# sea-sky-web/Vision-based-Spatio-Temporal-Analysis

Hardware: AMD Instinct MI355X
Metric: multi-cam frames/sec (7-cam→480×1440 BEV) (higher is better)
Workload: dtype f32; 1 GPU; 7-cam 1080x1920 -> resnet50(stride-8 features)+proj C=64 -> IPM warp -> mean -> 480x1440 BEV (BASELINE configs[1]); cameras=7, cameras_per_gpu=7, channels=64, bev_memory_format=NCHW, parallelism=frame-sharded x1 (no collective)

## Files before the change

### include/bev_mi355x.h

```cpp
#ifndef BEV_MI355X_H
#define BEV_MI355X_H

#include <stdint.h>

#ifdef __cplusplus
extern "C" {
#endif

#define BEV_ERR_ARGS (-1)

#define BEV_FUSE_SUM 0
#define BEV_FUSE_MEAN 1
#define BEV_FUSE_MAX 2

int bev_abi_version(void);

const char *bev_build_source_hash(void);

#define BEV_TUNE_CONV_TILE 1
#define BEV_TUNE_WARP_POOL_KB 2
#define BEV_TUNE_WARP_KERNEL 3
#define BEV_TUNE_WARP_BWD_POOL 5
#define BEV_TUNE_CONV_XCD 6
#define BEV_TUNE_CONV_NBUF 7
#define BEV_TUNE_WGRAD_MFMA 8
#define BEV_TUNE_CONV_DMA 9
#define BEV_TUNE_CONV_X6_TILE 10
#define BEV_TUNE_CONV_X6_KERNEL 11
#define BEV_TUNE_CONV_H16_KERNEL 12
#define BEV_TUNE_CONV_PW_SMALL 13
#define BEV_TUNE_DW_RUN 14
#define BEV_TUNE_CONV_X6_NT 16
#define BEV_TUNE_STEM3_STAGE 17
#define BEV_TUNE_WARP_SPAN 19
#define BEV_TUNE_WARP_TILE_BAND 20
#define BEV_TUNE_CONV_H16_BUF 21
#define BEV_TUNE_CONV_X6_STRIP 22
int bev_tune(int knob, int value);


int bev_linspace_f32(double lo, double hi, int n, float *out_host);

int bev_homography_f32(const float *K, const float *G, int n, float *H, void *stream);


int bev_ipm_warp_f32(const float *feats, int64_t sN, int64_t sC, int64_t sH, int64_t sW, const float *Hmat,
                     const float *xs, const float *ys, int N, int C, int Hf, int Wf, float sx, float sy, int Hb,
                     int Wb, float *out, void *stream);

int bev_ipm_warp_fuse_f32(const float *feats, int64_t sN, int64_t sC, int64_t sH, int64_t sW, const float *Hmat,
                          const float *xs, const float *ys, int B, int V, int C, int Hf, int Wf, float sx, float sy,
                          int Hb, int Wb, int mode, float *out, void *stream);
// ... 365 lines not shown
```

### vision-based-spatio-temporal-analysis_amd/bev_native.py

```python
from __future__ import annotations

import collections.abc
import contextlib
import ctypes
import functools
import os
import subprocess
import threading

import torch

HERE = os.path.dirname(os.path.abspath(__file__))
LIB_PATH = os.path.join(HERE, "libbev_mi355x.so")
ABI_VERSION = 18
BEV_ERR_ARGS = -1

FUSE_MODES = {"sum": 0, "mean": 1, "max": 2}

_lib = None

_vp = ctypes.c_void_p
_i = ctypes.c_int
_i64 = ctypes.c_int64
_f = ctypes.c_float
# ... 233 lines not shown
TUNE_CONV_XCD = 6
TUNE_CONV_NBUF = 7
TUNE_WGRAD_MFMA = 8
TUNE_CONV_DMA = 9
TUNE_CONV_X6_TILE = 10
TUNE_CONV_X6_KERNEL = 11
TUNE_CONV_H16_KERNEL = 12
TUNE_CONV_PW_SMALL = 13
TUNE_DW_RUN = 14
TUNE_CONV_X6_NT = 16
TUNE_STEM3_STAGE = 17
TUNE_WARP_SPAN = 19
TUNE_WARP_TILE_BAND = 20
TUNE_CONV_H16_BUF = 21
TUNE_CONV_X6_STRIP = 22
WARP_KERNEL_DMA, WARP_KERNEL_REGISTER = 0, 1


def tune(knob: int, value: int) -> int:
    rc = lib().bev_tune(knob, value)
    if rc < 0:
        raise ValueError(f"bad tuning knob/value {knob}/{value}")
    return rc


@contextlib.contextmanager
def tuned(**knobs):
    old = []
    try:
        for name, value in knobs.items():
# ... 1910 lines not shown
```

### vision-based-spatio-temporal-analysis_amd/csrc/bev_conv.hip

```cpp
#include <hip/hip_runtime.h>
#include <stdint.h>
#include <stdlib.h>

#include <type_traits>

#include "../../include/bev_mi355x.h"
#include "bev_act.h"
#include "bev_mfma.h"
#include "bev_tune.h"

namespace {

constexpr int BK = 32;
constexpr int LROW = BK + 4;

typedef float f32x16 __attribute__((ext_vector_type(16)));
typedef float f32x2 __attribute__((ext_vector_type(2)));
typedef float f32x4 __attribute__((ext_vector_type(4)));

__device__ __attribute__((aligned(16))) float g_zero4[4] = {0.f, 0.f, 0.f, 0.f};

__host__ __device__ inline int64_t kpad(int K) { return (K + BK - 1) / BK * BK; }
__host__ __device__ inline int64_t copad(int Co) { return (Co + 127) / 128 * 128; }

// ... 1258 lines not shown
    a.xcd = conv_xcd();
    return a;
}

}

extern "C" {

int bev_tune(int knob, int value) {
    if (knob == BEV_TUNE_CONV_TILE) return bev::swap_knob(g_conv_tile, value, 4);
    if (knob == BEV_TUNE_CONV_DMA) return bev::swap_knob(g_conv_dma, value, 2);
    if (knob == BEV_TUNE_CONV_XCD) return bev::swap_knob(g_conv_xcd, value, 1);
    if (knob == BEV_TUNE_CONV_NBUF) return bev::swap_knob(g_conv_nbuf, value, 2);
    if (knob == BEV_TUNE_WGRAD_MFMA) return bev::train_tune(knob, value);
    if (knob == BEV_TUNE_CONV_X6_TILE || knob == BEV_TUNE_CONV_X6_KERNEL || knob == BEV_TUNE_CONV_X6_NT ||
        knob == BEV_TUNE_CONV_X6_STRIP)
        return bev::conv_x6_tune(knob, value);
    if (knob == BEV_TUNE_CONV_H16_KERNEL) return bev::conv_h16_tune(value);
    if (knob == BEV_TUNE_CONV_H16_BUF) return bev::conv_h16_buf_tune(value);
    if (knob == BEV_TUNE_DW_RUN) return bev::dw_tune(value);
    if (knob == BEV_TUNE_STEM3_STAGE) return bev::stem3_tune(value);
    if (knob == BEV_TUNE_CONV_PW_SMALL) return bev::swap_knob(g_conv_pw_small, value, 4);
    return bev::warp_tune(knob, value);
}

int64_t bev_conv_packed_size(int Co, int Ci, int KH, int KW) {
    if (Co <= 0 || Ci <= 0 || KH <= 0 || KW <= 0) return 0;
    return copad(Co) * kpad(Ci * KH * KW);
}

int bev_conv_pack_weights_f32(const float *w, int Co, int Ci, int KH, int KW, float *packed, void *stream) {
// ... 237 lines not shown
```

### vision-based-spatio-temporal-analysis_amd/csrc/bev_conv_x6.hip

```cpp
#include <hip/hip_runtime.h>
#include <stdint.h>

#include <type_traits>

#include "../../include/bev_mi355x.h"
#include "bev_act.h"
#include "bev_mfma.h"
#include "bev_tune.h"

namespace {

typedef __bf16 bf16x8 __attribute__((ext_vector_type(8)));
typedef __bf16 bf16x4 __attribute__((ext_vector_type(4)));
typedef float f32x16 __attribute__((ext_vector_type(16)));
typedef float f32x4 __attribute__((ext_vector_type(4)));
typedef unsigned u32x4 __attribute__((ext_vector_type(4)));
typedef unsigned u32x2 __attribute__((ext_vector_type(2)));

constexpr int XBK = 16;
constexpr int XROW = 24;

__device__ __attribute__((aligned(16))) float g_xzero4[4] = {0.f, 0.f, 0.f, 0.f};

__host__ __device__ inline int64_t kpad_x(int K) { return (K + XBK - 1) / XBK * XBK; }
__host__ __device__ inline int64_t copad_x(int Co) { return (Co + 127) / 128 * 128; }

__device__ __forceinline__ void split3(float v, __bf16 &h, __bf16 &m, __bf16 &l) {
    h = (__bf16)v;
    const float r = v - (float)h;
    m = (__bf16)r;
    l = (__bf16)(r - (float)m);
}

__device__ __forceinline__ void x6_dot(f32x16 &c, const bf16x8 (&a)[3], const bf16x8 (&b)[3]) {
    c = __builtin_amdgcn_mfma_f32_32x32x16_bf16(a[0], b[0], c, 0, 0, 0);
    c = __builtin_amdgcn_mfma_f32_32x32x16_bf16(a[0], b[1], c, 0, 0, 0);
    c = __builtin_amdgcn_mfma_f32_32x32x16_bf16(a[1], b[0], c, 0, 0, 0);
    c = __builtin_amdgcn_mfma_f32_32x32x16_bf16(a[0], b[2], c, 0, 0, 0);
    c = __builtin_amdgcn_mfma_f32_32x32x16_bf16(a[2], b[0], c, 0, 0, 0);
    c = __builtin_amdgcn_mfma_f32_32x32x16_bf16(a[1], b[1], c, 0, 0, 0);
}

__host__ __device__ inline int64_t frag_index(int n, int k, int p, int64_t S) {
    return (((int64_t)(n >> 5) * S + (k >> 4)) * 3 + p) * 512 + (((k >> 3) & 1) * 32 + (n & 31)) * 8 + (k & 7);
}

// ... 97 lines not shown
            const int64_t mbase = m0 + wm * TM * 32 + i * 32;
            if (i > 0) res_load(i);
#pragma unroll
            for (int q = 0; q < NQ; ++q) {
                const int row = rq + RPI * q;
                const int64_t m = mbase + row;
                if (m >= a.M) continue;
                const float4 v = *(const float4 *)(E + row * ER + c4 * 4);
                float o[4] = {v.x + bv.x, v.y + bv.y, v.z + bv.z, v.w + bv.w};
                if (a.ys) {
                    if (a.res) {
                        const float4 rr = rv[q];
                        o[0] += rr.x, o[1] += rr.y, o[2] += rr.z, o[3] += rr.w;
                    }
                    bf16x4 hv, mv, lv;
#pragma unroll
                    for (int u = 0; u < 4; ++u) {
                        __bf16 h_, m_, l_;
                        split3(act_c<ACT>(o[u]), h_, m_, l_);
                        hv[u] = h_, mv[u] = m_, lv[u] = l_;
                    }
                    __bf16 *yp = a.ys + m * a.Co + n;
                    if (n < a.Co) {
                        *(bf16x4 *)yp = hv;
                        *(bf16x4 *)(yp + a.yps) = mv;
                        *(bf16x4 *)(yp + 2 * a.yps) = lv;
                    }
                    continue;
                }
                float *yp = a.y + m * a.ldy + n;
                if (nvec) {
                    if (a.res) {
                        o[0] += rv[q].x;
                        o[1] += rv[q].y;
                        o[2] += rv[q].z;
                        o[3] += rv[q].w;
// ... 3 lines not shown
                    *(float4 *)yp = make_float4(o[0], o[1], o[2], o[3]);
                } else {
#pragma unroll
                    for (int u = 0; u < 4; ++u) {
                        if (n + u >= a.Co) break;
                        float t = o[u];
                        if (a.res) t += a.res[m * a.Co + n + u];
                        yp[u] = act_c<ACT>(t);
                    }
                }
            }
        }
    });
}

template <int WM, int WN, int TM, int TN, bool DUAL>
__global__ __launch_bounds__(256, 2) void k_conv_x6(ConvX a) {
    constexpr int BM = WM * TM * 32, BN = WN * TN * 32;
    constexpr int APL = BM * XROW, BPL = BN * XROW;
    constexpr int STAGE = 3 * (APL + BPL);
    constexpr int AQ = BM / 64;
    constexpr int PB = ((BN * 6) % 256 == 0) ? 16 : 8;
    constexpr int PPR = 96 / PB;
    constexpr int BQ = BN * PPR / 256;
    static_assert(BN * PPR % 256 == 0, "B pieces per thread");
    typedef typename std::conditional<PB == 16, u32x4, u32x2>::type bpiece;
    constexpr int EPIB = x6_epi_bytes<TN>();
    constexpr int LDSB = (2 * STAGE * 2 > EPIB) ? 2 * STAGE * 2 : EPIB;
    static_assert(BM % 64 == 0, "A staging rows");
    __shared__ __attribute__((aligned(16))) unsigned char lds_raw[LDSB];
    __bf16 *lds = (__bf16 *)lds_raw;

    const int tid = threadIdx.x;
    const int lane = tid & 63, wave = __builtin_amdgcn_readfirstlane(tid >> 6);
    const int wm = wave / WN, wn = wave % WN;
    const int n_tiles = (a.Co + BN - 1) / BN;
    const unsigned bid = xcd_block(blockIdx.x, gridDim.x);
    const int64_t m0 = (int64_t)(bid / n_tiles) * BM;
    const int n0 = (bid % n_tiles) * BN;

    const int aq = tid & 3;
    int64_t pb[AQ], p2[AQ];
    int iy0[AQ], ix0[AQ];
    bool rok[AQ];
#pragma unroll
    for (int q = 0; q < AQ; ++q) {
        const int64_t m = m0 + (tid >> 2) + 64 * q;
        rok[q] = m < a.M;
        const int64_t mm = rok[q] ? m : 0;
        const int ox = (int)(mm % a.Wo);
        const int64_t t = mm / a.Wo;
        const int oy = (int)(t % a.Ho);
        const int64_t n = t / a.Ho;
        if (DUAL) {
            pb[q] = mm * a.Ci + 4 * aq;
            p2[q] = ((n * a.H2 + (int64_t)oy * a.stride2) * a.W2 + (int64_t)ox * a.stride2) * a.Ci2 + 4 * aq;
            iy0[q] = ix0[q] = 0;
        } else {
            pb[q] = n * a.H * a.W * a.Ci + 4 * aq;
            p2[q] = 0;
            iy0[q] = oy * a.stride - a.pad;
            ix0[q] = ox * a.stride - a.pad;
        }
    }
    const int64_t bstep = 3 * 512;
    const __bf16 *brow[BQ];
    int bdst[BQ];
#pragma unroll
    for (int i = 0; i < BQ; ++i) {
        const int pc = tid + 256 * i;
        const int row = pc / PPR, byte = (pc % PPR) * PB;
        const int pl = byte / 32, hk = (byte % 32) / 16, sub = (byte % 16) / 2;
        brow[i] = a.wp + frag_index(n0 + row, 8 * hk, pl, a.Kp / XBK) + sub;
        bdst[i] = pl * BPL + row * XROW + 8 * hk + sub;
    }
    f32x16 acc[TM][TN];
#pragma unroll
    for (int i = 0; i < TM; ++i)
#pragma unroll
        for (int j = 0; j < TN; ++j) acc[i][j] = (f32x16){0};

    f32x4 va0[AQ], va1[AQ];
    bpiece vb0[BQ], vb1[BQ];
    int ky = 0, kx = 0, ci0 = 0, k0 = 0;
    int64_t kb = 0;
#define X6_GLOAD(VA, VB)                                                                                   \
    do {                                                                                                   \
        if (DUAL) {                                                                                        \
            const bool first = k0 < a.Ci;                                                                  \
            const float *src = first ? a.x + k0 : a.x2 + (k0 - a.Ci);                                      \
            _Pragma("unroll") for (int q = 0; q < AQ; ++q) VA[q] =                                         \
                *(const f32x4 *)(rok[q] ? src + (first ? pb[q] : p2[q]) : g_xzero4);                      \
            k0 += XBK;                                                                                     \
        } else {                                                                                           \
            const int dy = ky * a.dil, dx = kx * a.dil;                                                    \
            _Pragma("unroll") for (int q = 0; q < AQ; ++q) {                                               \
                const int iy = iy0[q] + dy, ix = ix0[q] + dx;                                              \
                const bool in = rok[q] && (unsigned)iy < (unsigned)a.H && (unsigned)ix < (unsigned)a.W;    \
                VA[q] = *(const f32x4 *)(in ? a.x + pb[q] + ((int64_t)iy * a.W + ix) * a.Ci + ci0 : g_xzero4); \
            }                                                                                              \
            ci0 += XBK;                                                                                    \
            if (ci0 == a.Ci) {                                                                             \
// ... 1 lines not shown
                if (++kx == a.KW) {                                                                        \
                    kx = 0;                                                                                \
                    ++ky;                                                                                  \
                }                                                                                          \
            }                                                                                              \
        }                                                                                                  \
        _Pragma("unroll") for (int i = 0; i < BQ; ++i) VB[i] = *(const bpiece *)(brow[i] + kb);          \
        kb += bstep;                                                                                       \
    } while (0)
#define X6_SWRITE(BUF, VA, VB)                                                                             \
    do {                                                                                                   \
        __bf16 *As = lds + (BUF) * STAGE;                                                                  \
        __bf16 *Bs = As + 3 * APL;                                                                         \
        _Pragma("unroll") for (int q = 0; q < AQ; ++q) {                                                   \
            bf16x4 hv, mv, lv;                                                                             \
            _Pragma("unroll") for (int e = 0; e < 4; ++e) {                                                \
                __bf16 h_, m_, l_;                                                                         \
                split3(VA[q][e], h_, m_, l_);                                                              \
                hv[e] = h_;                                                                                \
                mv[e] = m_;                                                                                \
                lv[e] = l_;                                                                                \
            }                                                                                              \
            __bf16 *d = As + ((tid >> 2) + 64 * q) * XROW + 4 * aq;                                        \
            *(bf16x4 *)d = hv;                                                                             \
            *(bf16x4 *)(d + APL) = mv;                                                                     \
            *(bf16x4 *)(d + 2 * APL) = lv;                                                                 \
        }                                                                                                  \
        _Pragma("unroll") for (int i = 0; i < BQ; ++i) *(bpiece *)(Bs + bdst[i]) = VB[i];                \
    } while (0)
    const int r32 = lane & 31, h = lane >> 5;
#define X6_MFMA(BUF)                                                                                       \
    do {                                                                                                   \
        const __bf16 *As = lds + (BUF) * STAGE;                                                            \
        const __bf16 *Bs = As + 3 * APL;                                                                   \
        bf16x8 fa[TM][3], fb[TN][3];                                                                       \
        _Pragma("unroll") for (int i = 0; i < TM; ++i)                                                     \
            _Pragma("unroll") for (int p = 0; p < 3; ++p)                                                  \
// ... 99 lines not shown
        }
    };
    float rv[2][17];
    if (a.res) res_load(std::true_type{}, 32 * part, rv[0], true);
    else res_load(std::false_type{}, 32 * part, rv[0], true);
    __syncthreads();
    issue_w3(0, 0, HB);
    act_dispatch(a.act, [&](auto ac) {
#pragma unroll
        for (int i = 0; i < TM; ++i)
#pragma unroll
            for (int j = 0; j < TN; ++j) {
                const int col = wn * TN * 32 + j * 32 + r32;
                const float bj = a.bias ? a.bias[col] : 0.0f;
#pragma unroll
                for (int r = 0; r < 16; ++r) {
                    __bf16 h_, m_, l_;
                    split3(act_c<decltype(ac)::value>(acc[i][j][r] + bj), h_, m_, l_);
                    const int row = wm * TM * 32 + i * 32 + (r & 3) + 8 * (r >> 2) + 4 * hh;
                    H[row * HR + col] = h_;
                    H[HPL + row * HR + col] = m_;
                    H[2 * HPL + row * HR + col] = l_;
                }
            }
    });
    __syncthreads();
    bf16x8 fa[ST][3];
    {
        const __bf16 *ap = H + (band + r32) * HR + 8 * hh;
#pragma unroll
        for (int t = 0; t < S2; ++t)
#pragma unroll
            for (int p = 0; p < 3; ++p) fa[t][p] = *(const bf16x8 *)(ap + p * HPL + 16 * t);
    }
    if constexpr (X2S > 0) {
        int64_t m = m0 + band + r32;
        const bool ok = m < a.M;
// ... 64 lines not shown
        }
        for (int g = 0; g < NG; g += 2) {
            block(hr, a2, g, rv[0], rv[1]);
            if (g + 1 < NG) block(hr, a2, g + 1, rv[1], rv[0]);
        }
    };
    act_dispatch(a.act2, [&](auto a2) {
        if (a.res) run(std::true_type{}, a2);
        else run(std::false_type{}, a2);
    });
}

constexpr int YBK = 32;
constexpr int YROW = 40;

template <int WM, int WN, int TM, int TN, bool DUAL, int CHAIN = 0, bool NT = false>
__global__ __launch_bounds__(256, 2) void k_conv_x6b(ConvX a) {
    constexpr int BM = WM * TM * 32, BN = WN * TN * 32;
    constexpr int APL = BM * YROW;
    constexpr int STAGE = 3 * APL;
    constexpr int AQ = BM / 32;
    constexpr int EPIB = CHAIN ? x6_chain_lds_bytes<BM, BN>() : x6_epi_bytes<TN>();
    constexpr int LDSB = (2 * STAGE * 2 > EPIB) ? 2 * STAGE * 2 : EPIB;
    __shared__ __attribute__((aligned(16))) unsigned char lds_raw[LDSB];
    __bf16 *lds = (__bf16 *)lds_raw;

    const int tid = threadIdx.x;
    const int lane = tid & 63, wave = __builtin_amdgcn_readfirstlane(tid >> 6);
    const int wm = wave / WN, wn = wave % WN;
    const int n_tiles = (a.Co + BN - 1) / BN;
    const unsigned bid = xcd_block(blockIdx.x, gridDim.x);
    const int64_t m0 = (int64_t)(bid / n_tiles) * BM;
    const int n0 = (bid % n_tiles) * BN;

    const int aq = tid & 7;
    int64_t pb[AQ], p2[AQ];
    int iy0[AQ], ix0[AQ];
    bool rok[AQ];
#pragma unroll
    for (int q = 0; q < AQ; ++q) {
        const int64_t m = m0 + (tid >> 3) + 32 * q;
        rok[q] = m < a.M;
        const int64_t mm = rok[q] ? m : 0;
        const int ox = (int)(mm % a.Wo);
        const int64_t t = mm / a.Wo;
        const int oy = (int)(t % a.Ho);
        const int64_t n = t / a.Ho;
        if (DUAL) {
            pb[q] = mm * a.Ci + 4 * aq;
            p2[q] = ((n * a.H2 + (int64_t)oy * a.stride2) * a.W2 + (int64_t)ox * a.stride2) * a.Ci2 + 4 * aq;
            iy0[q] = ix0[q] = 0;
        } else {
            pb[q] = n * a.H * a.W * a.Ci + 4 * aq;
            p2[q] = 0;
            iy0[q] = oy * a.stride - a.pad;
            ix0[q] = ox * a.stride - a.pad;
        }
    }
    const int64_t S = a.Kp / XBK;
    const __bf16 *wb = a.wp + ((int64_t)((n0 + wn * TN * 32) >> 5) * S) * 1536 + lane * 8;
    const int nslice = a.Kp / XBK;

    f32x16 acc[TM][TN];
#pragma unroll
    for (int i = 0; i < TM; ++i)
#pragma unroll
        for (int j = 0; j < TN; ++j) acc[i][j] = (f32x16){0};

    f32x4 va0[AQ], va1[AQ];
    bf16x8 bs0[TN][3], bs1[TN][3];
    int ky = 0, kx = 0, ci0 = 0, k0 = 0;
#define X6B_GLOAD(VA)                                                                                      \
    do {                                                                                                   \
        if (DUAL) {                                                                                        \
            const bool first = k0 < a.Ci;                                                                  \
            const float *src = first ? a.x + k0 : a.x2 + (k0 - a.Ci);                                      \
            _Pragma("unroll") for (int q = 0; q < AQ; ++q) VA[q] =                                         \
                *(const f32x4 *)(rok[q] ? src + (first ? pb[q] : p2[q]) : g_xzero4);                      \
            k0 += YBK;                                                                                     \
        } else {                                                                                           \
            const int dy = ky * a.dil, dx = kx * a.dil;                                                    \
            _Pragma("unroll") for (int q = 0; q < AQ; ++q) {                                               \
                const int iy = iy0[q] + dy, ix = ix0[q] + dx;                                              \
                const bool in = rok[q] && (unsigned)iy < (unsigned)a.H && (unsigned)ix < (unsigned)a.W;    \
                const f32x4 *ap_ = (const f32x4 *)(in ? a.x + pb[q] + ((int64_t)iy * a.W + ix) * a.Ci + ci0 : g_xzero4); \
                if (NT) VA[q] = __builtin_nontemporal_load(ap_);                                          \
                else VA[q] = *ap_;                                                                        \
            }                                                                                              \
            ci0 += YBK;                                                                                    \
            if (ci0 == a.Ci) {                                                                             \
                ci0 = 0;                                                                                   \
                if (++kx == a.KW) {                                                                        \
                    kx = 0;                                                                                \
                    ++ky;                                                                                  \
                }                                                                                          \
            }                                                                                              \
        }                                                                                                  \
    } while (0)
#define X6B_SWRITE(BUF, VA)                                                                                \
    do {                                                                                                   \
        __bf16 *As = lds + (BUF) * STAGE;                                                                  \
        _Pragma("unroll") for (int q = 0; q < AQ; ++q) {                                                   \
            bf16x4 hv, mv, lv;                                                                             \
            _Pragma("unroll") for (int e = 0; e < 4; ++e) {                                                \
                __bf16 h_, m_, l_;                                                                         \
                split3(VA[q][e], h_, m_, l_);                                                              \
                hv[e] = h_;                                                                                \
                mv[e] = m_;                                                                                \
                lv[e] = l_;                                                                                \
            }                                                                                              \
            __bf16 *d = As + ((tid >> 3) + 32 * q) * YROW + 4 * aq;                                        \
            *(bf16x4 *)d = hv;                                                                             \
            *(bf16x4 *)(d + APL) = mv;                                                                     \
            *(bf16x4 *)(d + 2 * APL) = lv;                                                                 \
        }                                                                                                  \
    } while (0)
#define X6B_BLOAD(BS, G)                                                                                   \
    do {                                                                                                   \
        const int g_ = (G) < nslice ? (G) : nslice - 1;              \
        _Pragma("unroll") for (int j = 0; j < TN; ++j)                                                     \
            _Pragma("unroll") for (int p = 0; p < 3; ++p)                                                  \
                BS[j][p] = *(const bf16x8 *)(wb + ((int64_t)j * S + g_) * 1536 + p * 512);                \
    } while (0)
    const int r32 = lane & 31, h = lane >> 5;
#define X6B_SLICE(AS, KK, BC)                                                                              \
    do {                                                                                                   \
        bf16x8 fa[TM][3];                                                                                  \
        _Pragma("unroll") for (int i = 0; i < TM; ++i)                                                     \
            _Pragma("unroll") for (int p = 0; p < 3; ++p)                                                  \
                fa[i][p] = *(const bf16x8 *)(AS + p * APL + (wm * TM * 32 + i * 32 + r32) * YROW + 16 * (KK) + 8 * h); \
        _Pragma("unroll") for (int i = 0; i < TM; ++i)                                                     \
            _Pragma("unroll") for (int j = 0; j < TN; ++j)                                                 \
                x6_dot(acc[i][j], fa[i], BC[j]);                                                           \
    } while (0)
#define X6B_MFMA(BUF, KS)                                                                                  \
    do {                                                                                                   \
        const __bf16 *As = lds + (BUF) * STAGE;                                                            \
// ... 313 lines not shown
            X6S_SLICE(As, 1, bs1);
            asm volatile("s_waitcnt vmcnt(0)" ::: "memory");
            __syncthreads();
        }
    }
#undef X6S_SLICE
#undef X6S_BLOAD
    if constexpr (CHAIN > 0) {
        x6_chain_epilogue<WM, WN, TM, TN, CHAIN == 2 ? 4 : 0>(a, lds_raw, acc, wave, lane, wm, wn, m0);
        return;
    }
    x6_epilogue<TM, TN>(a, (float *)lds_raw, acc, wave, lane, wn, wm, m0, n0);
}

__global__ void k_split3(const float *__restrict__ x, int64_t n, __bf16 *__restrict__ out) {
    const int64_t t = (int64_t)blockIdx.x * blockDim.x + threadIdx.x;
    if (t >= n) return;
    __bf16 h, m, l;
    split3(x[t], h, m, l);
    out[t] = h;
    out[t + n] = m;
    out[t + 2 * n] = l;
}

int g_x6_tile = 0;
int g_x6_nt = 0;
int g_x6_kernel = 0;
int g_x6_strip = 1;

int launch_x6(void (*kernel)(ConvX), int BM, int BN, const ConvX &a, hipStream_t st) {
    const int64_t blocks = ((a.M + BM - 1) / BM) * ((a.Co + BN - 1) / BN);
    if (blocks >= ((int64_t)1 << 31)) return BEV_ERR_ARGS;
    hipLaunchKernelGGL(kernel, dim3((unsigned)blocks), dim3(256), 0, st, a);
    return last();
}

enum X6Form { X6_PLAIN, X6_DUAL, X6_CHAIN, X6_CHAIN_DUAL };
struct X6Call {
    X6Form form;
    const float *x = nullptr;
    const uint16_t *xs = nullptr, *packed = nullptr;
    const float *bias = nullptr, *res = nullptr;
    float *y = nullptr;
// ... 32 lines not shown
    if (c.form == X6_CHAIN && c.Co != 64 && c.Co2 % 128 != 0) return BEV_ERR_ARGS;

    ConvX a;
    a.x = c.x, a.wp = (const __bf16 *)c.packed, a.bias = c.bias, a.res = c.res, a.y = c.y;
    a.N = c.N, a.H = c.H, a.W = c.W, a.Ci = c.Ci, a.Co = c.Co, a.KH = c.KH, a.KW = c.KW, a.stride = c.stride;
    a.pad = c.pad, a.dil = c.dil, a.Ho = c.Ho, a.Wo = c.Wo, a.act = c.act, a.ldy = chain ? c.Co2 : c.ldy;
    a.Kp = (int)kpad_x(c.form == X6_DUAL ? c.Ci + c.Ci2 : c.Ci * c.KH * c.KW);
    a.M = (int64_t)c.N * c.Ho * c.Wo;
    a.x2 = c.x2, a.Ci2 = c.Ci2, a.H2 = c.H2, a.W2 = c.W2, a.stride2 = c.stride2;
    a.xs = (const __bf16 *)c.xs, a.ys = (__bf16 *)c.ys;
    a.xps = (int64_t)c.N * c.H * c.W * c.Ci, a.yps = a.M * c.Co;
    a.wp2 = (const __bf16 *)c.packed2, a.bias2 = c.bias2, a.Co2 = c.Co2, a.act2 = c.act2;

    const bool strip = g_x6_strip && c.xs && c.KH == 3 && c.KW == 3 && c.stride == 1 && c.pad == 1 && c.dil == 1 &&
                       c.Ci == 64;
    if (c.form == X6_CHAIN_DUAL && strip) return launch_x6(k_conv_x6s<4, 1, 1, 2, 2, true>, 128, 64, a, st);
    if (c.form == X6_CHAIN_DUAL)
        return launch_x6(c.xs ? k_conv_x6s<4, 1, 1, 2, 2> : k_conv_x6b<4, 1, 1, 2, false, 2>, 128, 64, a, st);
    if (c.form == X6_CHAIN && c.Co == 64 && strip) return launch_x6(k_conv_x6s<4, 1, 1, 2, 1, true>, 128, 64, a, st);
    if (c.form == X6_CHAIN && c.Co == 64)
        return launch_x6(c.xs ? k_conv_x6s<4, 1, 1, 2, 1> : k_conv_x6b<4, 1, 1, 2, false, 1>, 128, 64, a, st);
    if (c.form == X6_CHAIN)
        return launch_x6(c.xs ? k_conv_x6s<2, 2, 1, 2, 1> : k_conv_x6b<2, 2, 1, 2, false, 1>, 64, 128, a, st);
    const bool dual = c.form == X6_DUAL;
    a.nta = g_x6_nt;
    const int t = g_x6_tile ? g_x6_tile : (a.Co <= 64 ? 2 : 1);
    if (a.xs) return t == 2 ? launch_x6(k_conv_x6s<4, 1, 1, 2>, 128, 64, a, st)
                            : launch_x6(k_conv_x6s<2, 2, 2, 2>, 128, 128, a, st);
    const bool wide = a.Ci % YBK == 0 && (!dual || a.Ci2 % YBK == 0) && g_x6_kernel != 1;
    if (wide && t == 2 && !dual && a.nta) return launch_x6(k_conv_x6b<4, 1, 1, 2, false, 0, true>, 128, 64, a, st);
    if (wide && t == 2)
        return launch_x6(dual ? k_conv_x6b<4, 1, 1, 2, true> : k_conv_x6b<4, 1, 1, 2, false>, 128, 64, a, st);
    if (wide) return launch_x6(dual ? k_conv_x6b<2, 2, 2, 2, true> : k_conv_x6b<2, 2, 2, 2, false>, 128, 128, a, st);
    if (t == 2) return launch_x6(dual ? k_conv_x6<4, 1, 1, 2, true> : k_conv_x6<4, 1, 1, 2, false>, 128, 64, a, st);
    return launch_x6(dual ? k_conv_x6<2, 2, 2, 2, true> : k_conv_x6<2, 2, 2, 2, false>, 128, 128, a, st);
}

namespace stem6 {
constexpr int TW = 64, TH = 8, NTHR = 512;
constexpr int PR = 2 * TH + 5;
constexpr int PC = 2 * TW + 5;
constexpr int PITCH = 136;
constexpr int PLANE = 3 * PR * PITCH;
constexpr int PER_T = 17;
constexpr int NRUN = 3 * 7;
constexpr int NS = (NRUN + 2) / 2;
constexpr int WB = 2 * NS * 3 * 512;
constexpr int S_PANEL = 10;
__host__ __device__ constexpr int roff(int run) { return run >= NRUN ? 0 : ((run % 3) * PR + run / 3) * PITCH; }
static_assert(PITCH >= 2 * TW + 6 && PITCH % 2 == 0, "slot 7 of the last output column inside the row");
// ... 302 lines not shown
    a.nTx = (Wo + stem6::TW - 1) / stem6::TW;
    a.nTy = (Ho + stem6::TH - 1) / stem6::TH;
    a.ntiles = (int64_t)N * a.nTx * a.nTy;
    a.edge_b = a.edge_r = nullptr;
    a.Hp = a.Wp = 0;
    return a;
}
unsigned stem_x6_grid(const StemX6Args &a) { return (unsigned)(a.ntiles < cu_count() ? a.ntiles : cu_count()); }

}

namespace bev {
int conv_x6_tune(int knob, int value) {
    if (knob == BEV_TUNE_CONV_X6_TILE) return swap_knob(g_x6_tile, value, 2);
    if (knob == BEV_TUNE_CONV_X6_STRIP) return swap_knob(g_x6_strip, value, 1);
    return swap_knob(knob == BEV_TUNE_CONV_X6_NT ? g_x6_nt : g_x6_kernel, value, 1);
}
}

extern "C" {

int64_t bev_conv_packed_size_x6(int Co, int Ci, int KH, int KW) {
    if (Co <= 0 || Ci <= 0 || KH <= 0 || KW <= 0) return BEV_ERR_ARGS;
    return copad_x(Co) * kpad_x(Ci * KH * KW) * 3;
}

int bev_conv_pack_weights_x6(const float *w, int Co, int Ci, int KH, int KW, uint16_t *packed, void *stream) {
    if (!w || !packed || Co <= 0 || Ci <= 0 || KH <= 0 || KW <= 0) return BEV_ERR_ARGS;
    const int64_t Kp = kpad_x(Ci * KH * KW), Cop = copad_x(Co), n = Kp * Cop;
    hipLaunchKernelGGL(k_pack_x6, dim3((unsigned)((n + 255) / 256)), dim3(256), 0, (hipStream_t)stream, w, Co, Ci, KH,
// ... 2 lines not shown
}

int bev_conv2d_x6_f32(const float *x, const uint16_t *xs, int N, int H, int W, int Ci, const uint16_t *packed,
                      const float *bias, const float *residual, int Co, int KH, int KW, int stride, int pad,
                      int dilation, int act, float *y, uint16_t *ys, int ldy, int Ho, int Wo, void *stream) {
    X6Call c{X6_PLAIN};
    c.x = x, c.xs = xs, c.packed = packed, c.bias = bias, c.res = residual, c.y = y, c.ys = ys;
    c.N = N, c.H = H, c.W = W, c.Ci = Ci, c.Co = Co, c.KH = KH, c.KW = KW, c.stride = stride, c.pad = pad;
    c.dil = dilation, c.act = act, c.ldy = ldy, c.Ho = Ho, c.Wo = Wo;
    return conv_x6(c, (hipStream_t)stream);
}

int bev_split3_f32(const float *x, int64_t n, uint16_t *planes, void *stream) {
    if (!x || !planes || n < 0) return BEV_ERR_ARGS;
    if (n == 0) return 0;
    hipLaunchKernelGGL(k_split3, dim3((unsigned)((n + 255) / 256)), dim3(256), 0, (hipStream_t)stream, x, n,
                       (__bf16 *)planes);
    return last();
}

int bev_conv2d_dual_x6_f32(const float *x, int N, int Ho, int Wo, int Ci, const float *x2, int H2, int W2, int Ci2,
                           int stride2, const uint16_t *packed, const float *bias, int Co, int act, float *y,
                           void *stream) {
    X6Call c{X6_DUAL};
    c.x = x, c.packed = packed, c.bias = bias, c.y = y;
    c.N = N, c.H = c.Ho = Ho, c.W = c.Wo = Wo, c.Ci = Ci, c.Co = c.ldy = Co, c.act = act;
    c.x2 = x2, c.H2 = H2, c.W2 = W2, c.Ci2 = Ci2, c.stride2 = stride2;
    return conv_x6(c, (hipStream_t)stream);
}

int bev_conv2d_chain_x6_f32(const float *x, const uint16_t *xs, int N, int H, int W, int Ci,
// ... 64 lines not shown
```

Before: 142.2 frames/s.

## Use buffer-resource loads for x6 conv operand fetch and vectorize bf16 split

Adds templated BUFA variants of the x6 bf16-split conv kernels that fetch activations and packed weights through AMD buffer resource descriptors. Out-of-bounds taps are redirected to an invalid offset so the hardware returns zero, which replaces per-element pointer arithmetic and branchy padding checks. The three-way bf16 split is also vectorized into two-element conversions, and k_split3 now handles two elements per thread. The new path is on by default behind a tune knob and adds 32-bit offset range limits plus larger template instantiations and extra register use.

```diff
diff --git a/include/bev_mi355x.h b/include/bev_mi355x.h
--- a/include/bev_mi355x.h
+++ b/include/bev_mi355x.h
@@ -36,6 +36,7 @@
 #define BEV_TUNE_WARP_TILE_BAND 20
 #define BEV_TUNE_CONV_H16_BUF 21
 #define BEV_TUNE_CONV_X6_STRIP 22
+#define BEV_TUNE_CONV_X6_BUF 23
 int bev_tune(int knob, int value);
 
 
diff --git a/vision-based-spatio-temporal-analysis_amd/bev_native.py b/vision-based-spatio-temporal-analysis_amd/bev_native.py
--- a/vision-based-spatio-temporal-analysis_amd/bev_native.py
+++ b/vision-based-spatio-temporal-analysis_amd/bev_native.py
@@ -271,6 +271,7 @@
 TUNE_WARP_TILE_BAND = 20
 TUNE_CONV_H16_BUF = 21
 TUNE_CONV_X6_STRIP = 22
+TUNE_CONV_X6_BUF = 23
 WARP_KERNEL_DMA, WARP_KERNEL_REGISTER = 0, 1
 
 
diff --git a/vision-based-spatio-temporal-analysis_amd/csrc/bev_conv.hip b/vision-based-spatio-temporal-analysis_amd/csrc/bev_conv.hip
--- a/vision-based-spatio-temporal-analysis_amd/csrc/bev_conv.hip
+++ b/vision-based-spatio-temporal-analysis_amd/csrc/bev_conv.hip
@@ -1296,7 +1296,7 @@
     if (knob == BEV_TUNE_CONV_NBUF) return bev::swap_knob(g_conv_nbuf, value, 2);
     if (knob == BEV_TUNE_WGRAD_MFMA) return bev::train_tune(knob, value);
     if (knob == BEV_TUNE_CONV_X6_TILE || knob == BEV_TUNE_CONV_X6_KERNEL || knob == BEV_TUNE_CONV_X6_NT ||
-        knob == BEV_TUNE_CONV_X6_STRIP)
+        knob == BEV_TUNE_CONV_X6_STRIP || knob == BEV_TUNE_CONV_X6_BUF)
         return bev::conv_x6_tune(knob, value);
     if (knob == BEV_TUNE_CONV_H16_KERNEL) return bev::conv_h16_tune(value);
     if (knob == BEV_TUNE_CONV_H16_BUF) return bev::conv_h16_buf_tune(value);
diff --git a/vision-based-spatio-temporal-analysis_amd/csrc/bev_conv_x6.hip b/vision-based-spatio-temporal-analysis_amd/csrc/bev_conv_x6.hip
--- a/vision-based-spatio-temporal-analysis_amd/csrc/bev_conv_x6.hip
+++ b/vision-based-spatio-temporal-analysis_amd/csrc/bev_conv_x6.hip
@@ -1,6 +1,7 @@
 #include <hip/hip_runtime.h>
 #include <stdint.h>
 
+#include <algorithm>
 #include <type_traits>
 
 #include "../../include/bev_mi355x.h"
@@ -14,6 +15,8 @@
 typedef __bf16 bf16x4 __attribute__((ext_vector_type(4)));
 typedef float f32x16 __attribute__((ext_vector_type(16)));
 typedef float f32x4 __attribute__((ext_vector_type(4)));
+typedef float f32x2 __attribute__((ext_vector_type(2)));
+typedef __bf16 bf16x2 __attribute__((ext_vector_type(2)));
 typedef unsigned u32x4 __attribute__((ext_vector_type(4)));
 typedef unsigned u32x2 __attribute__((ext_vector_type(2)));
 
@@ -30,6 +33,36 @@
     const float r = v - (float)h;
     m = (__bf16)r;
     l = (__bf16)(r - (float)m);
+}
+
+__device__ __forceinline__ void split3x2(f32x2 v, bf16x2 &h, bf16x2 &m, bf16x2 &l) {
+    h = __builtin_convertvector(v, bf16x2);
+    const f32x2 r = v - __builtin_convertvector(h, f32x2);
+    m = __builtin_convertvector(r, bf16x2);
+    l = __builtin_convertvector(r - __builtin_convertvector(m, f32x2), bf16x2);
+}
+__device__ __forceinline__ void split3x4(f32x4 v, bf16x4 &h, bf16x4 &m, bf16x4 &l) {
+    bf16x2 h0, m0, l0, h1, m1, l1;
+    split3x2((f32x2){v[0], v[1]}, h0, m0, l0);
+    split3x2((f32x2){v[2], v[3]}, h1, m1, l1);
+    h = __builtin_shufflevector(h0, h1, 0, 1, 2, 3);
+    m = __builtin_shufflevector(m0, m1, 0, 1, 2, 3);
+    l = __builtin_shufflevector(l0, l1, 0, 1, 2, 3);
+}
+
+template <int PB>
+__device__ __forceinline__ auto x6_bload(__amdgpu_buffer_rsrc_t r, int vo, int so) {
+    if constexpr (PB == 16) return __builtin_amdgcn_raw_buffer_load_b128(r, vo, so, 0);
+    else return __builtin_amdgcn_raw_buffer_load_b64(r, vo, so, 0);
+}
+constexpr int X6_VOUT = (int)0x80000000;
+constexpr int64_t X6_BUF_MAX = ((int64_t)1 << 31) - 16;
+__device__ __forceinline__ __amdgpu_buffer_rsrc_t x6_rsrc(const void *p, int64_t bytes) {
+    const uint64_t u = (uint64_t)(uintptr_t)p;
+    const uint32_t lo = (uint32_t)__builtin_amdgcn_readfirstlane((int)(uint32_t)u);
+    const uint32_t hi = (uint32_t)__builtin_amdgcn_readfirstlane((int)(uint32_t)(u >> 32));
+    const int nb = __builtin_amdgcn_readfirstlane((int)(bytes < X6_BUF_MAX ? bytes : X6_BUF_MAX));
+    return __builtin_amdgcn_make_buffer_rsrc((void *)(uintptr_t)(((uint64_t)hi << 32) | lo), 0, nb, 0x00020000);
 }
 
 __device__ __forceinline__ void x6_dot(f32x16 &c, const bf16x8 (&a)[3], const bf16x8 (&b)[3]) {
@@ -157,12 +190,8 @@
                         o[0] += rr.x, o[1] += rr.y, o[2] += rr.z, o[3] += rr.w;
                     }
                     bf16x4 hv, mv, lv;
-#pragma unroll
-                    for (int u = 0; u < 4; ++u) {
-                        __bf16 h_, m_, l_;
-                        split3(act_c<ACT>(o[u]), h_, m_, l_);
-                        hv[u] = h_, mv[u] = m_, lv[u] = l_;
-                    }
+                    split3x4((f32x4){act_c<ACT>(o[0]), act_c<ACT>(o[1]), act_c<ACT>(o[2]), act_c<ACT>(o[3])}, hv, mv,
+                             lv);
                     __bf16 *yp = a.ys + m * a.Co + n;
                     if (n < a.Co) {
                         *(bf16x4 *)yp = hv;
@@ -196,7 +225,37 @@
     });
 }
 
-template <int WM, int WN, int TM, int TN, bool DUAL>
+struct X6Desc {
+    __amdgpu_buffer_rsrc_t rx, rx2;
+    int64_t n_first;
+    int xbias;
+    bool lin;
+};
+template <bool DUAL>
+__device__ __forceinline__ X6Desc x6_desc(const ConvX &a, int64_t m0) {
+    X6Desc d;
+    d.lin = DUAL || (a.KH == 1 && a.KW == 1 && a.stride == 1 && a.pad == 0);
+    d.n_first = 0;
+    d.xbias = 0;
+    if (d.lin) {
+        d.rx = x6_rsrc(a.x + m0 * a.Ci, (a.M - m0) * a.Ci * 4);
+    } else {
+        d.n_first = m0 / ((int64_t)a.Ho * a.Wo);
+        d.xbias = a.pad * (a.W + 1) * a.Ci * 4;
+        const int64_t img = (int64_t)a.H * a.W * a.Ci * 4;
+        d.rx = x6_rsrc((const char *)a.x + d.n_first * img - d.xbias, (a.N - d.n_first) * img + d.xbias);
+    }
+    if (DUAL) {
+        d.n_first = m0 / ((int64_t)a.Ho * a.Wo);
+        const int64_t img2 = (int64_t)a.H2 * a.W2 * a.Ci2 * 4;
+        d.rx2 = x6_rsrc((const char *)a.x2 + d.n_first * img2, (a.N - d.n_first) * img2);
+    } else {
+        d.rx2 = d.rx;
+    }
+    return d;
+}
+
+template <int WM, int WN, int TM, int TN, bool DUAL, bool BUFA = false>
 __global__ __launch_bounds__(256, 2) void k_conv_x6(ConvX a) {
     constexpr int BM = WM * TM * 32, BN = WN * TN * 32;
     constexpr int APL = BM * XROW, BPL = BN * XROW;
@@ -225,10 +284,23 @@
     int64_t pb[AQ], p2[AQ];
     int iy0[AQ], ix0[AQ];
     bool rok[AQ];
+    X6Desc dsc;
+    if constexpr (BUFA) dsc = x6_desc<DUAL>(a, m0);
+    unsigned vr[AQ], vr2[AQ];
+    int vo[AQ], vo2[AQ];
 #pragma unroll
     for (int q = 0; q < AQ; ++q) {
         const int64_t m = m0 + (tid >> 2) + 64 * q;
         rok[q] = m < a.M;
+        if constexpr (BUFA && !DUAL) {
+            if (dsc.lin) {
+                vr[q] = (unsigned)((tid >> 2) + 64 * q) * (unsigned)a.Ci * 4u + 16u * aq;
+                vr2[q] = 0;
+                iy0[q] = ix0[q] = 0;
+                pb[q] = p2[q] = 0;
+                continue;
+            }
+        }
         const int64_t mm = rok[q] ? m : 0;
         const int ox = (int)(mm % a.Wo);
         const int64_t t = mm / a.Wo;
@@ -244,9 +316,24 @@
             iy0[q] = oy * a.stride - a.pad;
             ix0[q] = ox * a.stride - a.pad;
         }
+        if constexpr (BUFA) {
+            const unsigned nr = (unsigned)(int)(n - dsc.n_first);
+            if (DUAL) {
+                vr[q] = (unsigned)(int)(m - m0) * (unsigned)a.Ci * 4u + 16u * aq;
+                vr2[q] = ((nr * a.H2 + (unsigned)(oy * a.stride2)) * a.W2 + (unsigned)(ox * a.stride2)) *
+                             (unsigned)a.Ci2 * 4u + 16u * aq;
+            } else {
+                vr[q] = ((nr * a.H + (unsigned)iy0[q]) * a.W + (unsigned)ix0[q]) * (unsigned)a.Ci * 4u + 16u * aq +
+                        (unsigned)dsc.xbias;
+                vr2[q] = 0;
+            }
+        }
     }
     const int64_t bstep = 3 * 512;
     const __bf16 *brow[BQ];
+    int bvo[BQ];
+    __amdgpu_buffer_rsrc_t rw;
+    if constexpr (BUFA) rw = x6_rsrc(a.wp, copad_x(a.Co) * (int64_t)a.Kp * 6);
     int bdst[BQ];
 #pragma unroll
     for (int i = 0; i < BQ; ++i) {
@@ -254,6 +341,7 @@
         const int row = pc / PPR, byte = (pc % PPR) * PB;
         const int pl = byte / 32, hk = (byte % 32) / 16, sub = (byte % 16) / 2;
         brow[i] = a.wp + frag_index(n0 + row, 8 * hk, pl, a.Kp / XBK) + sub;
+        bvo[i] = (int)((frag_index(n0 + row, 8 * hk, pl, a.Kp / XBK) + sub) * 2);
         bdst[i] = pl * BPL + row * XROW + 8 * hk + sub;
     }
     f32x16 acc[TM][TN];
@@ -266,8 +354,50 @@
     bpiece vb0[BQ], vb1[BQ];
     int ky = 0, kx = 0, ci0 = 0, k0 = 0;
     int64_t kb = 0;
+    int soff = 0;
+    auto x6_tap = [&]() {
+        const int dy = ky * a.dil, dx = kx * a.dil;
+        soff = (dy * a.W + dx) * a.Ci * 4;
+#pragma unroll
+        for (int q = 0; q < AQ; ++q) {
+            const int iy = iy0[q] + dy, ix = ix0[q] + dx;
+            const bool in = rok[q] & ((unsigned)iy < (unsigned)a.H) & ((unsigned)ix < (unsigned)a.W);
+            vo[q] = in ? (int)vr[q] : X6_VOUT;
+            vo2[q] = rok[q] ? (int)vr2[q] : X6_VOUT;
+        }
+    };
+    if constexpr (BUFA) x6_tap();
 #define X6_GLOAD(VA, VB)                                                                                   \
     do {                                                                                                   \
+        if constexpr (BUFA) {                                                                              \
+            if (DUAL) {                                                                                    \
+                if (k0 < a.Ci) {                                                                           \
+                    _Pragma("unroll") for (int q = 0; q < AQ; ++q) VA[q] = __builtin_bit_cast(             \
+                        f32x4, __builtin_amdgcn_raw_buffer_load_b128(dsc.rx, vo[q], k0 * 4, 0));           \
+                } else {                                                                                   \
+                    _Pragma("unroll") for (int q = 0; q < AQ; ++q) VA[q] = __builtin_bit_cast(             \
+                        f32x4, __builtin_amdgcn_raw_buffer_load_b128(dsc.rx2, vo2[q], (k0 - a.Ci) * 4, 0)); \
+                }                                                                                          \
+                k0 += XBK;                                                                                 \
+            } else {                                                                                       \
+                _Pragma("unroll") for (int q = 0; q < AQ; ++q) VA[q] = __builtin_bit_cast(                 \
+                    f32x4, __builtin_amdgcn_raw_buffer_load_b128(dsc.rx, vo[q], soff, 0));                 \
+                soff += XBK * 4;                                                                           \
+                ci0 += XBK;                                                                                \
+                if (ci0 == a.Ci) {                                                                         \
+                    ci0 = 0;                                                                               \
+                    if (++kx == a.KW) {                                                                    \
+                        kx = 0;                                                                            \
+                        ++ky;                                                                              \
+                    }                                                                                      \
+                    x6_tap();                                                                              \
+                }                                                                                          \
+            }                                                                                              \
+            _Pragma("unroll") for (int i = 0; i < BQ; ++i) VB[i] = __builtin_bit_cast(                     \
+                bpiece, x6_bload<PB>(rw, bvo[i], (int)kb * 2));                                            \
+            kb += bstep;                                                                                   \
+            break;                                                                                         \
+        }                                                                                                  \
         if (DUAL) {                                                                                        \
             const bool first = k0 < a.Ci;                                                                  \
             const float *src = first ? a.x + k0 : a.x2 + (k0 - a.Ci);                                      \
@@ -299,13 +429,7 @@
         __bf16 *Bs = As + 3 * APL;                                                                         \
         _Pragma("unroll") for (int q = 0; q < AQ; ++q) {                                                   \
             bf16x4 hv, mv, lv;                                                                             \
-            _Pragma("unroll") for (int e = 0; e < 4; ++e) {                                                \
-                __bf16 h_, m_, l_;                                                                         \
-                split3(VA[q][e], h_, m_, l_);                                                              \
-                hv[e] = h_;                                                                                \
-                mv[e] = m_;                                                                                \
-                lv[e] = l_;                                                                                \
-            }                                                                                              \
+            split3x4(VA[q], hv, mv, lv);                                                                   \
             __bf16 *d = As + ((tid >> 2) + 64 * q) * XROW + 4 * aq;                                        \
             *(bf16x4 *)d = hv;                                                                             \
             *(bf16x4 *)(d + APL) = mv;                                                                     \
@@ -435,13 +559,18 @@
                 const int col = wn * TN * 32 + j * 32 + r32;
                 const float bj = a.bias ? a.bias[col] : 0.0f;
 #pragma unroll
-                for (int r = 0; r < 16; ++r) {
-                    __bf16 h_, m_, l_;
-                    split3(act_c<decltype(ac)::value>(acc[i][j][r] + bj), h_, m_, l_);
-                    const int row = wm * TM * 32 + i * 32 + (r & 3) + 8 * (r >> 2) + 4 * hh;
-                    H[row * HR + col] = h_;
-                    H[HPL + row * HR + col] = m_;
-                    H[2 * HPL + row * HR + col] = l_;
+                for (int r = 0; r < 16; r += 2) {
+                    bf16x2 h_, m_, l_;
+                    split3x2((f32x2){act_c<decltype(ac)::value>(acc[i][j][r] + bj),
+                                     act_c<decltype(ac)::value>(acc[i][j][r + 1] + bj)},
+                             h_, m_, l_);
+#pragma unroll
+                    for (int e = 0; e < 2; ++e) {
+                        const int row = wm * TM * 32 + i * 32 + ((r + e) & 3) + 8 * ((r + e) >> 2) + 4 * hh;
+                        H[row * HR + col] = h_[e];
+                        H[HPL + row * HR + col] = m_[e];
+                        H[2 * HPL + row * HR + col] = l_[e];
+                    }
                 }
             }
     });
@@ -536,7 +665,7 @@
 constexpr int YBK = 32;
 constexpr int YROW = 40;
 
-template <int WM, int WN, int TM, int TN, bool DUAL, int CHAIN = 0, bool NT = false>
+template <int WM, int WN, int TM, int TN, bool DUAL, int CHAIN = 0, bool NT = false, bool BUFA = false>
 __global__ __launch_bounds__(256, 2) void k_conv_x6b(ConvX a) {
     constexpr int BM = WM * TM * 32, BN = WN * TN * 32;
     constexpr int APL = BM * YROW;
@@ -559,10 +688,23 @@
     int64_t pb[AQ], p2[AQ];
     int iy0[AQ], ix0[AQ];
     bool rok[AQ];
+    X6Desc dsc;
+    if constexpr (BUFA) dsc = x6_desc<DUAL>(a, m0);
+    unsigned vr[AQ], vr2[AQ];
+    int vo[AQ], vo2[AQ];
 #pragma unroll
     for (int q = 0; q < AQ; ++q) {
         const int64_t m = m0 + (tid >> 3) + 32 * q;
         rok[q] = m < a.M;
+        if constexpr (BUFA && !DUAL) {
+            if (dsc.lin) {
+                vr[q] = (unsigned)((tid >> 3) + 32 * q) * (unsigned)a.Ci * 4u + 16u * aq;
+                vr2[q] = 0;
+                iy0[q] = ix0[q] = 0;
+                pb[q] = p2[q] = 0;
+                continue;
+            }
+        }
         const int64_t mm = rok[q] ? m : 0;
         const int ox = (int)(mm % a.Wo);
         const int64_t t = mm / a.Wo;
@@ -578,10 +720,25 @@
             iy0[q] = oy * a.stride - a.pad;
             ix0[q] = ox * a.stride - a.pad;
         }
+        if constexpr (BUFA) {
+            const unsigned nr = (unsigned)(int)(n - dsc.n_first);
+            if (DUAL) {
+                vr[q] = (unsigned)(int)(m - m0) * (unsigned)a.Ci * 4u + 16u * aq;
+                vr2[q] = ((nr * a.H2 + (unsigned)(oy * a.stride2)) * a.W2 + (unsigned)(ox * a.stride2)) *
+                             (unsigned)a.Ci2 * 4u + 16u * aq;
+            } else {
+                vr[q] = ((nr * a.H + (unsigned)iy0[q]) * a.W + (unsigned)ix0[q]) * (unsigned)a.Ci * 4u + 16u * aq +
+                        (unsigned)dsc.xbias;
+                vr2[q] = 0;
+            }
+        }
     }
     const int64_t S = a.Kp / XBK;
     const __bf16 *wb = a.wp + ((int64_t)((n0 + wn * TN * 32) >> 5) * S) * 1536 + lane * 8;
     const int nslice = a.Kp / XBK;
+    __amdgpu_buffer_rsrc_t rw;
+    if constexpr (BUFA) rw = x6_rsrc(a.wp, copad_x(a.Co) / 32 * (int64_t)nslice * 3072);
+    const int cb0 = (n0 + wn * TN * 32) >> 5;
 
     f32x16 acc[TM][TN];
 #pragma unroll
@@ -592,8 +749,48 @@
     f32x4 va0[AQ], va1[AQ];
     bf16x8 bs0[TN][3], bs1[TN][3];
     int ky = 0, kx = 0, ci0 = 0, k0 = 0;
+    int soff = 0;
+    auto x6_tap = [&]() {
+        const int dy = ky * a.dil, dx = kx * a.dil;
+        soff = (dy * a.W + dx) * a.Ci * 4;
+#pragma unroll
+        for (int q = 0; q < AQ; ++q) {
+            const int iy = iy0[q] + dy, ix = ix0[q] + dx;
+            const bool in = rok[q] & ((unsigned)iy < (unsigned)a.H) & ((unsigned)ix < (unsigned)a.W);
+            vo[q] = in ? (int)vr[q] : X6_VOUT;
+            vo2[q] = rok[q] ? (int)vr2[q] : X6_VOUT;
+        }
+    };
+    if constexpr (BUFA) x6_tap();
+    constexpr int AUX = NT ? 2 : 0;
 #define X6B_GLOAD(VA)                                                                                      \
     do {                                                                                                   \
+        if constexpr (BUFA) {                                                                              \
+            if (DUAL) {                                                                                    \
+                if (k0 < a.Ci) {                                                                           \
+                    _Pragma("unroll") for (int q = 0; q < AQ; ++q) VA[q] = __builtin_bit_cast(             \
+                        f32x4, __builtin_amdgcn_raw_buffer_load_b128(dsc.rx, vo[q], k0 * 4, AUX));         \
+                } else {                                                                                   \
+                    _Pragma("unroll") for (int q = 0; q < AQ; ++q) VA[q] = __builtin_bit_cast(             \
+                        f32x4, __builtin_amdgcn_raw_buffer_load_b128(dsc.rx2, vo2[q], (k0 - a.Ci) * 4, AUX)); \
+                }                                                                                          \
+                k0 += YBK;                                                                                 \
+            } else {                                                                                       \
+                _Pragma("unroll") for (int q = 0; q < AQ; ++q) VA[q] = __builtin_bit_cast(                 \
+                    f32x4, __builtin_amdgcn_raw_buffer_load_b128(dsc.rx, vo[q], soff, AUX));               \
+                soff += YBK * 4;                                                                           \
+                ci0 += YBK;                                                                                \
+                if (ci0 == a.Ci) {                                                                         \
+                    ci0 = 0;                                                                               \
+                    if (++kx == a.KW) {                                                                    \
+                        kx = 0;                                                                            \
+                        ++ky;                                                                              \
+                    }                                                                                      \
+                    x6_tap();                                                                              \
+                }                                                                                          \
+            }                                                                                              \
+            break;                                                                                         \
+        }                                                                                                  \
         if (DUAL) {                                                                                        \
             const bool first = k0 < a.Ci;                                                                  \
             const float *src = first ? a.x + k0 : a.x2 + (k0 - a.Ci);                                      \
@@ -624,13 +821,7 @@
         __bf16 *As = lds + (BUF) * STAGE;                                                                  \
         _Pragma("unroll") for (int q = 0; q < AQ; ++q) {                                                   \
             bf16x4 hv, mv, lv;                                                                             \
-            _Pragma("unroll") for (int e = 0; e < 4; ++e) {                                                \
-                __bf16 h_, m_, l_;                                                                         \
-                split3(VA[q][e], h_, m_, l_);                                                              \
-                hv[e] = h_;                                                                                \
-                mv[e] = m_;                                                                                \
-                lv[e] = l_;                                                                                \
-            }                                                                                              \
+            split3x4(VA[q], hv, mv, lv);                                                                   \
             __bf16 *d = As + ((tid >> 3) + 32 * q) * YROW + 4 * aq;                                        \
             *(bf16x4 *)d = hv;                                                                             \
             *(bf16x4 *)(d + APL) = mv;                                                                     \
@@ -641,8 +832,12 @@
     do {                                                                                                   \
         const int g_ = (G) < nslice ? (G) : nslice - 1;              \
         _Pragma("unroll") for (int j = 0; j < TN; ++j)                                                     \
-            _Pragma("unroll") for (int p = 0; p < 3; ++p)                                                  \
-                BS[j][p] = *(const bf16x8 *)(wb + ((int64_t)j * S + g_) * 1536 + p * 512);                \
+            _Pragma("unroll") for (int p = 0; p < 3; ++p) {                                                \
+                if constexpr (BUFA)                                                                        \
+                    BS[j][p] = __builtin_bit_cast(bf16x8, __builtin_amdgcn_raw_buffer_load_b128(           \
+                                                              rw, lane * 16, (((cb0 + j) * nslice + g_) * 3 + p) * 1024, 0)); \
+                else BS[j][p] = *(const bf16x8 *)(wb + ((int64_t)j * S + g_) * 1536 + p * 512);           \
+            }                                                                                              \
     } while (0)
     const int r32 = lane & 31, h = lane >> 5;
 #define X6B_SLICE(AS, KK, BC)                                                                              \
@@ -986,19 +1181,26 @@
 }
 
 __global__ void k_split3(const float *__restrict__ x, int64_t n, __bf16 *__restrict__ out) {
-    const int64_t t = (int64_t)blockIdx.x * blockDim.x + threadIdx.x;
+    const int64_t t = 2 * ((int64_t)blockIdx.x * blockDim.x + threadIdx.x);
     if (t >= n) return;
-    __bf16 h, m, l;
-    split3(x[t], h, m, l);
-    out[t] = h;
-    out[t + n] = m;
-    out[t + 2 * n] = l;
+    const bool two = t + 1 < n;
+    bf16x2 h, m, l;
+    split3x2((f32x2){x[t], two ? x[t + 1] : 0.0f}, h, m, l);
+    out[t] = h[0];
+    out[t + n] = m[0];
+    out[t + 2 * n] = l[0];
+    if (two) {
+        out[t + 1] = h[1];
+        out[t + 1 + n] = m[1];
+        out[t + 1 + 2 * n] = l[1];
+    }
 }
 
 int g_x6_tile = 0;
 int g_x6_nt = 0;
 int g_x6_kernel = 0;
 int g_x6_strip = 1;
+int g_x6_buf = 1;
 
 int launch_x6(void (*kernel)(ConvX), int BM, int BN, const ConvX &a, hipStream_t st) {
     const int64_t blocks = ((a.M + BM - 1) / BM) * ((a.Co + BN - 1) / BN);
@@ -1061,26 +1263,44 @@
 
     const bool strip = g_x6_strip && c.xs && c.KH == 3 && c.KW == 3 && c.stride == 1 && c.pad == 1 && c.dil == 1 &&
                        c.Ci == 64;
+    const int64_t span = std::min<int64_t>(c.N, 128 / ((int64_t)c.Ho * c.Wo) + 2);
+    const int64_t kp2 = kpad_x(c.form == X6_DUAL ? c.Ci + c.Ci2 : c.Ci * c.KH * c.KW);
+    const bool buf = g_x6_buf && c.x &&
+                     span * c.H * c.W * c.Ci * 4 + (int64_t)c.pad * (c.W + 1) * c.Ci * 4 < X6_BUF_MAX &&
+                     (!second || span * c.H2 * c.W2 * c.Ci2 * 4 < X6_BUF_MAX) &&
+                     copad_x(c.Co) * kp2 * 6 < ((int64_t)1 << 31);
+#define X6_PICK(K, ...) (buf ? K<__VA_ARGS__, true> : K<__VA_ARGS__, false>)
     if (c.form == X6_CHAIN_DUAL && strip) return launch_x6(k_conv_x6s<4, 1, 1, 2, 2, true>, 128, 64, a, st);
     if (c.form == X6_CHAIN_DUAL)
-        return launch_x6(c.xs ? k_conv_x6s<4, 1, 1, 2, 2> : k_conv_x6b<4, 1, 1, 2, false, 2>, 128, 64, a, st);
+        return launch_x6(c.xs ? k_conv_x6s<4, 1, 1, 2, 2> : X6_PICK(k_conv_x6b, 4, 1, 1, 2, false, 2, false), 128, 64, a,
+                         st);
     if (c.form == X6_CHAIN && c.Co == 64 && strip) return launch_x6(k_conv_x6s<4, 1, 1, 2, 1, true>, 128, 64, a, st);
     if (c.form == X6_CHAIN && c.Co == 64)
-        return launch_x6(c.xs ? k_conv_x6s<4, 1, 1, 2, 1> : k_conv_x6b<4, 1, 1, 2, false, 1>, 128, 64, a, st);
+        return launch_x6(c.xs ? k_conv_x6s<4, 1, 1, 2, 1> : X6_PICK(k_conv_x6b, 4, 1, 1, 2, false, 1, false), 128, 64, a,
+                         st);
     if (c.form == X6_CHAIN)
-        return launch_x6(c.xs ? k_conv_x6s<2, 2, 1, 2, 1> : k_conv_x6b<2, 2, 1, 2, false, 1>, 64, 128, a, st);
+        return launch_x6(c.xs ? k_conv_x6s<2, 2, 1, 2, 1> : X6_PICK(k_conv_x6b, 2, 2, 1, 2, false, 1, false), 64, 128, a,
+                         st);
     const bool dual = c.form == X6_DUAL;
     a.nta = g_x6_nt;
     const int t = g_x6_tile ? g_x6_tile : (a.Co <= 64 ? 2 : 1);
     if (a.xs) return t == 2 ? launch_x6(k_conv_x6s<4, 1, 1, 2>, 128, 64, a, st)
                             : launch_x6(k_conv_x6s<2, 2, 2, 2>, 128, 128, a, st);
     const bool wide = a.Ci % YBK == 0 && (!dual || a.Ci2 % YBK == 0) && g_x6_kernel != 1;
-    if (wide && t == 2 && !dual && a.nta) return launch_x6(k_conv_x6b<4, 1, 1, 2, false, 0, true>, 128, 64, a, st);
+    if (wide && t == 2 && !dual && a.nta)
+        return launch_x6(X6_PICK(k_conv_x6b, 4, 1, 1, 2, false, 0, true), 128, 64, a, st);
     if (wide && t == 2)
-        return launch_x6(dual ? k_conv_x6b<4, 1, 1, 2, true> : k_conv_x6b<4, 1, 1, 2, false>, 128, 64, a, st);
-    if (wide) return launch_x6(dual ? k_conv_x6b<2, 2, 2, 2, true> : k_conv_x6b<2, 2, 2, 2, false>, 128, 128, a, st);
-    if (t == 2) return launch_x6(dual ? k_conv_x6<4, 1, 1, 2, true> : k_conv_x6<4, 1, 1, 2, false>, 128, 64, a, st);
-    return launch_x6(dual ? k_conv_x6<2, 2, 2, 2, true> : k_conv_x6<2, 2, 2, 2, false>, 128, 128, a, st);
+        return launch_x6(dual ? X6_PICK(k_conv_x6b, 4, 1, 1, 2, true, 0, false)
+                              : X6_PICK(k_conv_x6b, 4, 1, 1, 2, false, 0, false), 128, 64, a, st);
+    if (wide)
+        return launch_x6(dual ? X6_PICK(k_conv_x6b, 2, 2, 2, 2, true, 0, false)
+                              : X6_PICK(k_conv_x6b, 2, 2, 2, 2, false, 0, false), 128, 128, a, st);
+    if (t == 2)
+        return launch_x6(dual ? X6_PICK(k_conv_x6, 4, 1, 1, 2, true) : X6_PICK(k_conv_x6, 4, 1, 1, 2, false), 128, 64,
+                         a, st);
+    return launch_x6(dual ? X6_PICK(k_conv_x6, 2, 2, 2, 2, true) : X6_PICK(k_conv_x6, 2, 2, 2, 2, false), 128, 128, a,
+                     st);
+#undef X6_PICK
 }
 
 namespace stem6 {
@@ -1413,6 +1633,7 @@
 int conv_x6_tune(int knob, int value) {
     if (knob == BEV_TUNE_CONV_X6_TILE) return swap_knob(g_x6_tile, value, 2);
     if (knob == BEV_TUNE_CONV_X6_STRIP) return swap_knob(g_x6_strip, value, 1);
+    if (knob == BEV_TUNE_CONV_X6_BUF) return swap_knob(g_x6_buf, value, 1);
     return swap_knob(knob == BEV_TUNE_CONV_X6_NT ? g_x6_nt : g_x6_kernel, value, 1);
 }
 }
@@ -1445,7 +1666,7 @@
 int bev_split3_f32(const float *x, int64_t n, uint16_t *planes, void *stream) {
     if (!x || !planes || n < 0) return BEV_ERR_ARGS;
     if (n == 0) return 0;
-    hipLaunchKernelGGL(k_split3, dim3((unsigned)((n + 255) / 256)), dim3(256), 0, (hipStream_t)stream, x, n,
+    hipLaunchKernelGGL(k_split3, dim3((unsigned)((n + 511) / 512)), dim3(256), 0, (hipStream_t)stream, x, n,
                        (__bf16 *)planes);
     return last();
 }
```

Measured after the change: 144.1 frames/s (median of 6 runs). +1.3%, better.
